# reedrosenbluth/LASS

Measured on AMD Instinct MI355X. Metric: clips/sec (10s@16kHz), higher is better.
Workload: dtype f32; 1 GPU; ResUNet30 separate() fp32, batch=16/GPU, 10s@16kHz clips, fixed precomputed condition embedding, seeded random-init weights (BASELINE configs[1]); samples_per_clip=160000, parallelism=clip-sharded x1

## Files before the change

### include/lass_hip.h

```cpp
#ifndef LASS_HIP_H
#define LASS_HIP_H

#include <stddef.h>
#include <stdint.h>

#ifdef __cplusplus
extern "C" {
#endif

typedef struct lass_ctx lass_ctx;

#define LASS_OK 0
#define LASS_ERR_ARG (-1)
#define LASS_ERR_HIP (-2)
#define LASS_ERR_STATE (-3)
#define LASS_ERR_WORKSPACE (-4)

#define LASS_F32 0
#define LASS_I64 1

#define LASS_COMPUTE_F32 0
#define LASS_COMPUTE_BF16 1
#define LASS_COMPUTE_BF16X3 2

// ... 8 lines not shown

const char* lass_last_error(const lass_ctx* ctx);

int lass_set_param(lass_ctx* ctx, const char* name, const void* data, const int64_t* shape, int ndim, int dtype);

int lass_finalize(lass_ctx* ctx, int compute_mode);

int lass_workspace_bytes(const lass_ctx* ctx, int B, int L, size_t* bytes);

int lass_separate(lass_ctx* ctx, const float* mixture, const float* condition, float* out, int B, int L,
                  void* workspace, size_t workspace_bytes, void* stream);


int lass_separate_ragged(lass_ctx* ctx, const float* mixture, const int* lengths, const float* condition, float* out,
                         int B, int L, void* workspace, size_t workspace_bytes, void* stream);
int lass_ragged_bucket(const lass_ctx* ctx, int L, int* lo, int* hi);


int lass_separate_windows(lass_ctx* ctx, const float* recording, int64_t total, const int64_t* starts, const int* keep,
                          const float* condition , float* out , int B, int W,
                          void* workspace, size_t workspace_bytes, void* stream);

int lass_separate_windows_faded(lass_ctx* ctx, const float* recording, int64_t total, const int64_t* starts, const int* keep,
                                const int* fade, const float* ramp, int F, const float* condition ,
                                float* out , int B, int W, void* workspace, size_t workspace_bytes, void* stream);

int lass_graph_stats(const lass_ctx* ctx, long* captures, long* replays);
int lass_set_graph_replay(lass_ctx* ctx, int enabled);
int lass_set_wino4_splits(lass_ctx* ctx, int splits);
int lass_set_wino4_vprep(lass_ctx* ctx, int mode);
int lass_set_head_fold(lass_ctx* ctx, int enabled);
int lass_set_head_sc_fold(lass_ctx* ctx, int enabled);
int lass_set_pw_split(lass_ctx* ctx, int enabled);
int lass_set_wino4_gemm(lass_ctx* ctx, int enabled);
int lass_set_wino4_vprep_buffer(lass_ctx* ctx, float* v, size_t floats);

int lass_separate_components(lass_ctx* ctx, const float* const* mag, const float* cos_mask, const float* sin_mask,
                             const float* condition, float* out, int B, int L, void* workspace, size_t workspace_bytes,
                             void* stream);


int lass_stft_magphase(lass_ctx* ctx, const float* wav, int B, int L, float* mag, float* cos_out, float* sin_out,
                       float* real_out, float* imag_out, void* stream);

int lass_multi_stft(lass_ctx* ctx, const float* wav, int B, int L, int hop, int n_windows, const int* win_lengths,
                    float* const* mag, float* const* cos_out, float* const* sin_out, void* stream);

int lass_stft_components(lass_ctx* ctx, const float* wav, int B, int L, int n_fft, int hop, int n_windows,
                         const int* win_lengths, float* const* mag, float* const* cos_out, float* const* sin_out,
                         void* stream);

int lass_istft(lass_ctx* ctx, const float* real, const float* imag, int B, int T, int L, float* wav,
               float* frames_ws, void* stream);
int lass_istft_nfft(lass_ctx* ctx, const float* real, const float* imag, int B, int T, int L, int n_fft, int win_length,
                    float* wav, void* stream);

int lass_film(lass_ctx* ctx, const float* condition, int B, float* shift, void* stream);
int lass_film_width(const lass_ctx* ctx);
int lass_film_offset(const lass_ctx* ctx, const char* site);
int lass_film_raw(lass_ctx* ctx, const float* condition, int B, float* film, void* stream);

int lass_convblock(lass_ctx* ctx, const char* prefix, const float* x, int B, int H, int W, const float* shift,
                   float* y, float* scratch, void* stream);

int lass_encoder_block(lass_ctx* ctx, const char* name, const float* x, int B, int H, int W, const float* shift, float* y,
                       float* pool, float* scratch, void* stream);
// ... 122 lines not shown
```

### lass_amd/_lib.py

```python
from __future__ import annotations

import ctypes
import os
from ctypes import POINTER, c_char_p, c_double, c_float, c_int, c_int64, c_long, c_size_t, c_void_p

_HERE = os.path.dirname(os.path.abspath(__file__))
LIB_PATH = os.environ.get("LASS_HIP_LIB") or os.path.join(_HERE, "csrc", "liblass_hip.so")

_lib = None

SYMBOLS = [
    ("lass_version", c_int, []),
    ("lass_create", c_int, [POINTER(c_void_p), c_int]),
    ("lass_create_stft", c_int, [POINTER(c_void_p), c_int, c_int, c_int]),
    ("lass_stft_geometry", c_int, [c_void_p, POINTER(c_int), POINTER(c_int)]),
    ("lass_create_multistft", c_int, [POINTER(c_void_p), c_int, c_int, c_int, POINTER(c_int), c_int]),
    ("lass_destroy", c_int, [c_void_p]),
    ("lass_last_error", c_char_p, [c_void_p]),
    ("lass_set_param", c_int, [c_void_p, c_char_p, c_void_p, POINTER(c_int64), c_int, c_int]),
    ("lass_finalize", c_int, [c_void_p, c_int]),
    ("lass_workspace_bytes", c_int, [c_void_p, c_int, c_int, POINTER(c_size_t)]),
    ("lass_separate", c_int, [c_void_p, c_void_p, c_void_p, c_void_p, c_int, c_int, c_void_p, c_size_t, c_void_p]),
    ("lass_separate_ragged", c_int, [c_void_p, c_void_p, c_void_p, c_void_p, c_void_p, c_int, c_int, c_void_p, c_size_t,
                                     c_void_p]),
# ... 14 lines not shown
                                         c_int, c_int, c_int, c_int, c_int, c_void_p, c_void_p]),
    ("lass_stft_magphase", c_int, [c_void_p, c_void_p, c_int, c_int, c_void_p, c_void_p, c_void_p, c_void_p,
                                   c_void_p, c_void_p]),
    ("lass_mix_at_snr", c_int, [c_void_p, c_void_p, c_void_p, c_void_p, c_void_p, c_int, c_int, c_void_p, c_void_p]),
    ("lass_decode_resample", c_int, [c_void_p, c_void_p, c_int64, c_int, c_int, c_int, c_int, c_int, c_int, c_void_p, c_int,
                                     c_void_p, c_int, c_void_p]),
    ("lass_decode_resample_planar", c_int, [c_void_p, c_void_p, c_int64, c_int, c_int, c_int, c_int, c_int, c_int, c_void_p, c_int,
                                            c_void_p, c_int, c_void_p]),
    ("lass_resample_encode", c_int, [c_void_p, c_void_p, c_int64, c_int64, c_int, c_int, c_int, c_int, c_int, c_void_p, c_int, c_int,
                                     c_void_p, c_int64, c_int, c_void_p, c_void_p]),
    ("lass_loudness", c_int, [c_void_p, c_void_p, c_int64, c_int64, c_int, c_int, c_int, c_void_p, c_int, POINTER(c_double), c_void_p,
                              c_void_p, c_void_p, c_int, c_void_p, c_size_t, c_void_p]),
    ("lass_resample_peak", c_int, [c_void_p, c_void_p, c_int64, c_int64, c_int, c_int, c_int, c_int, c_int, c_void_p, c_int, c_int,
                                   c_void_p, c_void_p]),
    ("lass_loudness_gain", c_int, [c_void_p, c_void_p, c_void_p, c_int, c_double, c_float, c_void_p, c_void_p, c_void_p]),
    ("lass_resample_encode_gain", c_int, [c_void_p, c_void_p, c_int64, c_int64, c_int, c_int, c_int, c_int, c_int, c_void_p, c_int,
                                          c_int, c_void_p, c_void_p, c_int64, c_int, c_void_p, c_void_p]),
    ("lass_resample_true_peak", c_int, [c_void_p, c_void_p, c_int64, c_int64, c_int, c_int, c_int, c_int, c_int, c_void_p, c_int, c_int,
                                        c_int, c_void_p, c_int, c_void_p, c_void_p]),
    ("lass_loudness_stats", c_int, [c_void_p, c_void_p, c_int64, c_int64, c_int, c_int, c_int, c_void_p, c_int, POINTER(c_double),
                                    c_void_p, c_void_p, c_void_p, c_int, c_void_p, c_int, c_void_p, c_size_t, c_void_p]),
    ("lass_segment_mix", c_int, [c_void_p, c_void_p, c_int, c_int, c_void_p, c_void_p, c_int, c_void_p, c_void_p, c_void_p,
                                 c_void_p, c_void_p]),
    ("lass_multi_stft", c_int, [c_void_p, c_void_p, c_int, c_int, c_int, c_int, POINTER(c_int), POINTER(c_void_p),
                                POINTER(c_void_p), POINTER(c_void_p), c_void_p]),
    ("lass_graph_stats", c_int, [c_void_p, POINTER(c_long), POINTER(c_long)]),
    ("lass_set_graph_replay", c_int, [c_void_p, c_int]),
    ("lass_set_wino4_splits", c_int, [c_void_p, c_int]),
    ("lass_set_wino4_vprep", c_int, [c_void_p, c_int]),
    ("lass_set_wino4_vprep_buffer", c_int, [c_void_p, c_void_p, c_size_t]),
    ("lass_set_head_fold", c_int, [c_void_p, c_int]),
    ("lass_set_head_sc_fold", c_int, [c_void_p, c_int]),
    ("lass_set_pw_split", c_int, [c_void_p, c_int]),
    ("lass_set_wino4_gemm", c_int, [c_void_p, c_int]),
    ("lass_separate_components", c_int, [c_void_p, POINTER(c_void_p), c_void_p, c_void_p, c_void_p, c_void_p, c_int,
                                         c_int, c_void_p, c_size_t, c_void_p]),
    ("lass_stft_components", c_int, [c_void_p, c_void_p, c_int, c_int, c_int, c_int, c_int, POINTER(c_int),
                                     POINTER(c_void_p), POINTER(c_void_p), POINTER(c_void_p), c_void_p]),
    ("lass_istft_nfft", c_int, [c_void_p, c_void_p, c_void_p, c_int, c_int, c_int, c_int, c_int, c_void_p, c_void_p]),
    ("lass_istft", c_int, [c_void_p, c_void_p, c_void_p, c_int, c_int, c_int, c_void_p, c_void_p, c_void_p]),
    ("lass_film", c_int, [c_void_p, c_void_p, c_int, c_void_p, c_void_p]),
    ("lass_film_width", c_int, [c_void_p]),
    ("lass_film_offset", c_int, [c_void_p, c_char_p]),
    ("lass_film_raw", c_int, [c_void_p, c_void_p, c_int, c_void_p, c_void_p]),
    ("lass_convblock", c_int, [c_void_p, c_char_p, c_void_p, c_int, c_int, c_int, c_void_p, c_void_p, c_void_p,
                               c_void_p]),
    ("lass_encoder_block", c_int, [c_void_p, c_char_p, c_void_p, c_int, c_int, c_int, c_void_p, c_void_p, c_void_p,
                                   c_void_p, c_void_p]),
    ("lass_front_end", c_int, [c_void_p, c_void_p, c_int, c_int, c_void_p, c_void_p, c_void_p, c_void_p, c_void_p]),
    ("lass_workspace_tensor", c_int, [c_void_p, c_int, c_int, c_char_p, POINTER(c_size_t), POINTER(c_int64),
                                      POINTER(c_int64)]),
    ("lass_upconv", c_int, [c_void_p, c_char_p, c_void_p, c_int, c_int, c_int, c_void_p, c_void_p, c_void_p]),
    ("lass_mask_apply", c_int, [c_void_p, c_void_p, c_void_p, c_void_p, c_void_p, c_int, c_int, c_int, c_void_p,
                                c_void_p, c_void_p]),
    ("lass_sdr_stats", c_int, [c_void_p, c_void_p, c_void_p, c_int, c_int, c_void_p, c_void_p]),
    ("lass_text_create", c_int, [POINTER(c_void_p), c_int]),
    ("lass_text_destroy", c_int, [c_void_p]),
    ("lass_text_last_error", c_char_p, [c_void_p]),
    ("lass_text_set_param", c_int, [c_void_p, c_char_p, c_void_p, POINTER(c_int64), c_int]),
    ("lass_text_finalize", c_int, [c_void_p]),
    ("lass_text_layers", c_int, [c_void_p]),
    ("lass_text_workspace_bytes", c_int, [c_void_p, c_int, c_int, POINTER(c_size_t)]),
    ("lass_text_encode", c_int, [c_void_p, c_void_p, c_void_p, c_int, c_int, c_void_p, c_void_p, c_void_p, c_size_t,
                                 c_void_p]),
    ("lass_audioq_create", c_int, [POINTER(c_void_p), c_int]),
    ("lass_audioq_destroy", c_int, [c_void_p]),
# ... 99 lines not shown
```

### lass_amd/csrc/api.hip

```cpp
#include <hip/hip_runtime.h>

#include <algorithm>
#include <cmath>
#include <cstdio>
#include <cstdlib>
#include <cstring>
#include <map>
#include <string>
#include <vector>

#include "../../include/lass_hip.h"
#include "ctx_parts.h"
#include "graph_cache.h"
#include "head_fold.h"
#include "kernels.h"
#include "weight_plan.h"
#include "workspace_plan.h"

namespace {

constexpr float kBnEps = 1e-5f;
constexpr int kMaxBranches = LASS_MAX_STFT_WINDOWS;

struct Site {
// ... 359 lines not shown
                            : form == BF16_DEC6U && f.up && lass_dec6u_fused_bf16_supported(p, q, uq)))
        return fail(c, LASS_ERR_STATE, rb.prefix + ": the launch arguments contradict the planned route");
    ProfScope ps(c, st, P_CONV3X3);
    HIP_TRY(c, form == BF16_ENC1 ? lass_launch_enc1_fused_bf16(p, q, st) : form == BF16_DEC6 ? lass_launch_dec6_fused_bf16(p, q, st)
                                 : lass_launch_dec6u_fused_bf16(p, q, uq, st));
    return 0;
}

int launch_routed(lass_ctx* c, const ResBlock& rb, const char* what, const ConvRoute& rt, const ConvArgs& a, const Wino4Split& sk,
                  float* vws, const Wino4Gemm& wg, hipStream_t st, const HeadScPlanes* planes = nullptr) {
    ProfScope ps(c, st, P_CONV3X3);
    bool ok = true;
    switch (rt.family) {
        case CONV_F4X4: {
            const Wino4Split s = rt.splits > 1 ? sk : Wino4Split();
            Wino4VPre vp;
            if (rt.v_from_memory) vp.v = vws;
            if (rt.head_sc_fold) {
                ok = planes && (rt.head_fold ? lass_wino4_headfold_planes_supported(a, *planes) : lass_wino4_sclogit_supported(a, *planes));
                if (ok) HIP_TRY(c, rt.head_fold ? lass_launch_wino4_headfold_planes(a, *planes, st) : lass_launch_wino4_sclogit(a, *planes, st));
                break;
            }
            if (rt.head_fold) {
                ok = lass_wino4_headfold_supported(a);
                if (ok) HIP_TRY(c, lass_launch_wino4_headfold(a, st));
                break;
            }
            if (rt.gemm) {
                ok = lass_wino4_gemm_supported(rt.kind, a, vp, wg);
                if (ok) HIP_TRY(c, lass_launch_wino4_gemm(rt.kind, a, vp, wg, st));
                break;
            }
            ok = rt.v_from_memory ? lass_wino4_vpre_supported(rt.kind, a, s) : lass_wino4_supported(rt.kind, a, s);
            if (ok) HIP_TRY(c, lass_launch_wino4(rt.kind, a, st, s, vp));
            break;
        }
        case CONV_F2X2:
            ok = lass_wino_supported(a);
            if (ok) HIP_TRY(c, lass_launch_wino(rt.kind, a, st));
            break;
        case CONV_DIRECT:
            HIP_TRY(c, lass_launch_conv(rt.kind, a, st));
            break;
        case CONV_NONE:
            ok = false;
            break;
    }
    return ok ? 0 : fail(c, LASS_ERR_STATE, rb.prefix + " " + what + ": the launch arguments contradict the planned route");
}

int run_resblock(lass_ctx* c, const ResBlock& rb, const float* x, long x_bs, int B, int H, int W, const float* shift,
                 float* a2, float* out, long out_bs, hipStream_t st, const BlockFusions& f = BlockFusions()) {
    const PreConv* pre = f.pre;
    const WeightImages& im = rb.img;
    const CatCopies *skip_out = f.skip_out, *cat_in = f.cat_in, *pool_copies = f.pool_copies;
    const float* x0 = pre ? pre->x0 : nullptr;
    const Site& s1 = c->sites[rb.s1];
    const Site& s2 = c->sites[rb.s2];
    const long HW = (long)H * W;
    ConvArgs p;
    p.in = x; p.in_bs = x_bs; p.Cin = rb.cin; p.w = im.f32(W1); p.Nw = rb.cout; p.N = rb.cout;
    p.pro_scale = c->bn_scale + s1.off; p.pro_shift = shift + s1.off; p.pro_shift_bs = c->n_shift;
    p.epi_scale = c->bn_scale + s2.off; p.epi_shift = shift + s2.off; p.epi_shift_bs = c->n_shift;
    p.out = a2; p.out_bs = rb.cout * HW; p.B = B; p.H = H; p.W = W;
    if (x0) {
        p.in = x0; p.in_bs = HW;
        p.pre_w = pre->w; p.pre_b = pre->b;
// ... 239 lines not shown

struct HeadHost {
    HeadFold hf;
    HeadScFold hsf;
    const std::vector<float>& of(WeightForm f) const {
        return f == WF_HEAD_U4 ? hf.u4 : f == WF_HEAD_WSC ? hf.wsc : f == WF_HEAD_BIAS ? hf.bias : f == WF_HEAD_SC_WT ? hsf.wt : hsf.wskip;
    }
};
int compose_head(lass_ctx* c, int Q, bool sc, HeadHost* h) {
    const ResBlock& rb = c->dec[5];
    const DecSpec& d6 = c->m.D[5];
    const int N = rb.cout, K = rb.cin;
    std::vector<float> w2, ws, bs, wa, ba, wt;
    const auto host = [&](std::vector<float>& v, const std::string& name, size_t n) -> int {
        v.resize(n);
        HIP_TRY(c, hipMemcpy(v.data(), rawp(c, name), n * sizeof(float), hipMemcpyDeviceToHost));
        return 0;
    };
    HIP_TRY(c, hipStreamSynchronize(nullptr));
    if (host(w2, rb.prefix + ".conv2.weight", (size_t)N * N * 9) || host(ws, rb.prefix + ".shortcut.weight", (size_t)N * K) ||
        host(bs, rb.prefix + ".shortcut.bias", N) || host(wa, "base.after_conv.weight", (size_t)Q * N) ||
        host(ba, "base.after_conv.bias", Q) ||
        (sc && host(wt, std::string("base.") + d6.name + ".conv1.weight", (size_t)d6.cin * d6.cout * d6.uh * d6.uw)))
        return LASS_ERR_HIP;
    if (sc) compose_head_sc_fold(ws.data(), wa.data(), wt.data(), N, d6.cout, kPreCh, Q, d6.cin, d6.uh, d6.uw, &h->hsf);
    if (!compose_head_fold(w2.data(), ws.data(), bs.data(), wa.data(), ba.data(), N, N, K, Q, &h->hf) || h->hf.u4.empty()) h->hf = HeadFold();
    return 0;
}

}

extern "C" {

int lass_version(void) { return 10900; }

const char* lass_last_error(const lass_ctx* ctx) { return ctx ? ctx->err.c_str() : g_create_err.c_str(); }

static int create_impl(lass_ctx** out, int device_id, const Geometry& geom) {
    if (!out) return LASS_ERR_ARG;
    *out = nullptr;
    if (int rc = open_device(device_id, g_create_err)) return rc;
    lass_ctx* c = new lass_ctx();
    c->device = device_id;
    c->g = geom;
    if (const char* e = getenv("LASS_FUSE_CATB")) c->cfg.fuse_catb = atoi(e) != 0;
    if (const char* e = getenv("LASS_FUSE_BLOCK")) c->cfg.fuse_block = atoi(e) != 0;
    if (const char* e = getenv("LASS_FUSE_UP")) c->cfg.fuse_up = atoi(e) != 0;
    if (const char* e = getenv("LASS_WINO4")) c->cfg.wino4_mincin = atoi(e);
    if (const char* e = getenv("LASS_WINO4_VPREP")) c->cfg.vprep_mode = std::max(0, std::min(2, atoi(e)));
    if (const char* e = getenv("LASS_HEAD_FOLD")) c->cfg.head_fold = atoi(e) != 0;
    if (const char* e = getenv("LASS_HEAD_SC_FOLD")) c->cfg.head_sc_fold = atoi(e) != 0;
    if (const char* e = getenv("LASS_PW_SPLIT")) c->cfg.pw_split = atoi(e) != 0;
    if (const char* e = getenv("LASS_WINO4_GEMM")) c->cfg.wino4_gemm = atoi(e) != 0;
    if (const char* e = getenv("LASS_SPLIT")) c->split_batch = std::max(0, std::min(2, atoi(e)));
    if (const char* e = getenv("LASS_GRAPH")) c->use_graph = atoi(e) != 0;
    c->prof.resize(P_COUNT);
    for (int i = 0; i < P_COUNT; ++i) c->prof[i].name = kProfNames[i];
    build_arch(c);
    if (hipSetDevice(device_id) != hipSuccess) {
        g_create_err = "hipSetDevice failed";
        delete c;
        return LASS_ERR_HIP;
    }
    std::vector<float2> tw2k(2048);
    for (int k = 0; k < 2048; ++k) {
        const double a = 2.0 * M_PI * k / 2048.0;
        tw2k[k] = make_float2((float)std::cos(a), (float)std::sin(a));
    }
    if (hipMalloc((void**)&c->tw2k, sizeof(float2) * 2048) != hipSuccess ||
        hipMemcpy(c->tw2k, tw2k.data(), sizeof(float2) * 2048, hipMemcpyHostToDevice) != hipSuccess) {
        g_create_err = "allocating FFT tables failed";
        delete c;
        return LASS_ERR_HIP;
    }
    *out = c;
    return 0;
}

int lass_create(lass_ctx** out, int device_id) { return create_impl(out, device_id, Geometry()); }

int lass_create_stft(lass_ctx** out, int device_id, int n_fft, int hop) {
    if (!out) return LASS_ERR_ARG;
    *out = nullptr;
    Geometry g;
    if (n_fft == 2048 && hop == 320) {
// ... 1006 lines not shown
    c->cfg.ksplit_force = splits;
    ++c->gen;
    return 0;
}

int lass_set_wino4_vprep(lass_ctx* c, int mode) {
    if (!c || mode < 0 || mode > 2) return fail(c, LASS_ERR_ARG, "lass_set_wino4_vprep: 0, 1 or 2");
    c->cfg.vprep_mode = mode;
    ++c->gen;
    return 0;
}

int lass_set_head_fold(lass_ctx* c, int enabled) {
    if (!c || (enabled != 0 && enabled != 1)) return fail(c, LASS_ERR_ARG, "lass_set_head_fold: 0 or 1");
    c->cfg.head_fold = enabled != 0;
    ++c->gen;
    return 0;
}

int lass_set_head_sc_fold(lass_ctx* c, int enabled) {
    if (!c || (enabled != 0 && enabled != 1)) return fail(c, LASS_ERR_ARG, "lass_set_head_sc_fold: 0 or 1");
    c->cfg.head_sc_fold = enabled != 0;
    ++c->gen;
    return 0;
}

int lass_set_pw_split(lass_ctx* c, int enabled) {
    if (!c || (enabled != 0 && enabled != 1)) return fail(c, LASS_ERR_ARG, "lass_set_pw_split: 0 or 1");
    c->cfg.pw_split = enabled != 0;
    ++c->gen;
    return 0;
}

int lass_set_wino4_gemm(lass_ctx* c, int enabled) {
    if (!c || (enabled != 0 && enabled != 1)) return fail(c, LASS_ERR_ARG, "lass_set_wino4_gemm: 0 or 1");
    c->cfg.wino4_gemm = enabled != 0;
    ++c->gen;
    return 0;
}

int lass_set_wino4_vprep_buffer(lass_ctx* c, float* v, size_t floats) {
    if (!c || (v && !floats)) return fail(c, LASS_ERR_ARG, "lass_set_wino4_vprep_buffer: a buffer and its size, or NULL");
    c->stage_v_user = v;
    c->stage_v_user_floats = v ? floats : 0;
    return 0;
}

int lass_graph_stats(const lass_ctx* c, long* captures, long* replays) {
    if (!c) return LASS_ERR_ARG;
    if (captures) *captures = c->g_captures;
    if (replays) *replays = c->g_replays;
    return c->use_graph ? 1 : 0;
}

int lass_separate_components(lass_ctx* c, const float* const* mag, const float* cos_mask, const float* sin_mask,
                             const float* condition, float* out, int B, int L, void* workspace, size_t workspace_bytes,
                             void* stream) {
    if (!c) return LASS_ERR_ARG;
    if (!mag || !cos_mask || !sin_mask) return fail(c, LASS_ERR_ARG, "lass_separate_components: null pointer");
    Components comp;
    for (int k = 0; k < kMaxBranches; ++k) comp.mag[k] = k < c->g.nbr ? mag[k] : nullptr;
    comp.cosv = cos_mask; comp.sinv = sin_mask;
    return separate_impl(c, nullptr, &comp, condition, out, ClipForm{B, L}, make_plan(c, B, L), workspace, workspace_bytes, stream,
                         "lass_separate_components");
}

// ... 32 lines not shown
```

### lass_amd/csrc/conv_route.h

```cpp
#pragma once
#include <stddef.h>

enum ConvKind { CONV1_ACT = 0, CONV2_IDENT = 1, CONV2_SHORTCUT = 2, TCONV_ACT = 3, CONV1_ACT_PRE = 4, CONV2_IDENT_PRE = 5 };

constexpr int kPreCh = 32;

constexpr int kWinoKC = 8;
constexpr int kWino4KC = 8;
constexpr int kWino4NXI = 36;
constexpr int kWino4VFloats = kWino4NXI * 4 * 32 * 2;
constexpr int kHeadFoldRows = 16;
constexpr int kPwGemmNB = 128;
constexpr int kPwGemmKC = 16;
constexpr int kBf16FusedTileW = 32;

inline bool lass_wino4_narrow(int H, int W) { return W % 32 == 16 && H % 32 == 0; }
inline int lass_wino4_block_tc(int H, int W) {
    if (W % 64 == 0 && H % 8 == 0) return 16;
    if (W % 32 == 0 && H % 16 == 0) return 8;
    return lass_wino4_narrow(H, W) ? 4 : 0;
}

struct ConvShape {
    int Cin = 0, N = 0, Nw = 0, H = 0, W = 0;
// ... 75 lines not shown
}
inline bool lass_dec6u_fused_bf16_shape(const ConvShape& p, const ConvShape& q, int u_cin, int u_h, int u_w) {
    return lass_dec6_fused_bf16_shape(p, q) && u_cin == 64 && u_h * 2 == p.H && u_w * 2 == p.W && p.H % 2 == 0 &&
           lass_bf16_fused_addressable(u_h, u_w);
}

constexpr int kWino4Splits = 4;

constexpr int kShortcutGemmMinCin = 256;

constexpr int kVprepMinCoutGroups = 12;

constexpr int kTconvGemmMinCin = 128;

inline bool lass_pw_split_shortcut_weights(bool f32, int cin, int cout) {
    return f32 && cin != cout && cin >= kShortcutGemmMinCin && cin % (2 * kPwGemmKC) == 0 && cout % kPwGemmNB == 0;
}
inline bool lass_pw_split_tconv_weights(bool f32, int cin, int N, int up_h) {
    return f32 && cin >= kTconvGemmMinCin && cin % (2 * kPwGemmKC) == 0 && N % kPwGemmNB == 0 && (up_h == 1 || up_h == 2) && N % (2 * up_h) == 0;
}

enum ComputeMode { MODE_F32 = 0, MODE_BF16 = 1, MODE_BF16X3 = 2 };

struct RouteCfg {
    ComputeMode mode = MODE_F32;
    bool f32() const { return mode == MODE_F32; }
    int wino4_mincin = 32;
    int ksplit_force = 0;
    int vprep_mode = 1;
    bool head_fold = true;
    bool head_sc_fold = true;
    bool wino4_gemm = true;
    bool pw_split = true;
    bool fuse_catb = true;
    bool fuse_block = true;
    bool fuse_up = true;
    bool blocked() const { return mode == MODE_BF16 && fuse_catb; }
};

struct BlockShape {
    int cin, cout;
    int width;
};

struct BlockIO {
    bool x0 = false;
    bool head = false;
    bool pool = false;
    int pool_h = 2;
    bool x_aligned = true;
    bool sc_planes = false;
    bool cat_in = false;
    bool skip_out = false;
    bool pool_copies = false;
    bool act_out = false;
    int up_cin = 0;
};

struct Wino4Images {
    bool u1f = false, u2f = false;
};
inline Wino4Images wino4_images(const RouteCfg& cfg, int cin, int cout, int width) {
    Wino4Images im;
    const int m = cfg.wino4_mincin;
    if (!cfg.f32() || m <= 0 || cin % 8 != 0 || cout % 32 != 0) return im;
    const bool level = width % 32 == 0, narrow = width % 32 == 16;
// ... 345 lines not shown
```

### lass_amd/csrc/kernels.h

```cpp
#pragma once
#include <hip/hip_runtime.h>
#include <stddef.h>
#include <stdint.h>

#include "conv_route.h"

struct ConvArgs {
    const float* in = nullptr;
    long in_bs = 0;
    int Cin = 0;
    const float* w = nullptr;
    int Nw = 0;
    const float* pro_scale = nullptr;
    const float* pro_shift = nullptr;
    int pro_shift_bs = 0;
    const float* in2 = nullptr;
    long in2_bs = 0;
    int Cin2 = 0;
    const float* w2 = nullptr;
    const float* bias = nullptr;
    const float* res = nullptr;
    long res_bs = 0;
    const float* epi_scale = nullptr;
    const float* epi_shift = nullptr;
// ... 48 lines not shown
struct Wino4Split {
    int n = 1;
    float* part = nullptr;
};

struct Wino4VPre {
    float* v = nullptr;
};

struct HeadScPlanes {
    float* skip = nullptr;
    float* up = nullptr;
    const float* w = nullptr;
};

inline ConvShape lass_conv_shape(const ConvArgs& p) {
    ConvShape s;
    s.Cin = p.Cin; s.N = p.N; s.Nw = p.Nw; s.H = p.H; s.W = p.W;
    s.Cin2 = p.Cin2; s.pool = p.pool_out != nullptr; s.pool_h = p.pool_h; s.head = p.mask_re != nullptr;
    return s;
}

hipError_t lass_launch_conv(ConvKind kind, const ConvArgs& p, hipStream_t stream);
bool lass_tconv_logits_supported(const ConvArgs& p, const HeadScPlanes& hs);
hipError_t lass_launch_tconv_logits(const ConvArgs& p, const HeadScPlanes& hs, hipStream_t stream);

bool lass_wino_supported(const ConvArgs& p);
hipError_t lass_launch_wino(ConvKind kind, const ConvArgs& p, hipStream_t stream);
hipError_t lass_launch_wino_weights(const float* w, int Cout, int Cin, float* U, hipStream_t stream);
hipError_t lass_launch_wino_shortcut_weights(const float* w, int Cout, int Cin, float* U, hipStream_t stream);

bool lass_wino4_supported(ConvKind kind, const ConvArgs& p, const Wino4Split& sk = Wino4Split());
hipError_t lass_launch_wino4(ConvKind kind, const ConvArgs& p, hipStream_t stream, const Wino4Split& sk = Wino4Split(),
                             const Wino4VPre& vp = Wino4VPre());
bool lass_wino4_vpre_supported(ConvKind kind, const ConvArgs& p, const Wino4Split& sk = Wino4Split());
hipError_t lass_launch_wino4_weights(const float* w, int Cout, int Cin, float* U, hipStream_t stream);
bool lass_wino4_headfold_supported(const ConvArgs& p);
hipError_t lass_launch_wino4_headfold(const ConvArgs& p, hipStream_t stream);
bool lass_wino4_headfold_planes_supported(const ConvArgs& p, const HeadScPlanes& hs);
hipError_t lass_launch_wino4_headfold_planes(const ConvArgs& p, const HeadScPlanes& hs, hipStream_t stream);
bool lass_wino4_sclogit_supported(const ConvArgs& p, const HeadScPlanes& hs);
hipError_t lass_launch_wino4_sclogit(const ConvArgs& p, const HeadScPlanes& hs, hipStream_t stream);

struct Wino4Gemm {
    const void* w3 = nullptr;
    float* m = nullptr;
};
bool lass_wino4_gemm_supported(ConvKind kind, const ConvArgs& p, const Wino4VPre& vp, const Wino4Gemm& g);
hipError_t lass_launch_wino4_gemm(ConvKind kind, const ConvArgs& p, const Wino4VPre& vp, const Wino4Gemm& g, hipStream_t stream);
hipError_t lass_launch_wino4_gemm_weights(const float* U, int Cout, int Cin, void* dst, hipStream_t stream);

struct PwSplitW {
    const void* w = nullptr;
};
bool lass_pw_gemm_supported(ConvKind kind, const ConvArgs& p);
hipError_t lass_launch_pw_gemm(ConvKind kind, const ConvArgs& p, hipStream_t stream, const PwSplitW& sw = PwSplitW());
hipError_t lass_launch_pw_split_weights(const float* w, int K, int Nw, void* dst, hipStream_t stream);

bool lass_bf16_supported(const ConvArgs& p);
hipError_t lass_launch_conv_bf16(ConvKind kind, const ConvArgs& p, hipStream_t stream);
hipError_t lass_launch_weights_bf16(const float* w, int Cout, int Cin, int taps, void* dst, int lo, int transposed,
                                    hipStream_t stream);

bool lass_enc1_fused_bf16_supported(const ConvArgs& p, const ConvArgs& q);
hipError_t lass_launch_enc1_fused_bf16(const ConvArgs& p, const ConvArgs& q, hipStream_t stream);
bool lass_dec6_fused_bf16_supported(const ConvArgs& p, const ConvArgs& q);
hipError_t lass_launch_dec6_fused_bf16(const ConvArgs& p, const ConvArgs& q, hipStream_t stream);
// ... 83 lines not shown
```

### lass_amd/csrc/pw_gemm_split.h

```cpp
#pragma once
#include <hip/hip_runtime.h>
#include "kernels.h"
#include "pixel_ops.h"
#include "wino_common.h"

namespace {

constexpr int NTHREADS = 256;
constexpr int NB = kPwGemmNB;
constexpr int PB = 128;
constexpr int KC = kPwGemmKC;

typedef float f32x16 __attribute__((ext_vector_type(16)));

template <bool TCONV>
__device__ __forceinline__ void acc_init(const ConvArgs& p, f32x16 (&acc)[2][2], int n0, int wn, int lane) {
#pragma unroll
    for (int i = 0; i < 2; ++i)
#pragma unroll
        for (int r = 0; r < 16; ++r) {
            const float v = TCONV ? 0.f : p.bias[n0 + wn * 64 + i * 32 + 4 * (lane >> 5) + (r & 3) + 8 * (r >> 2)];
            acc[i][0][r] = v;
            acc[i][1][r] = v;
        }
}

__device__ __forceinline__ void acc_zero(f32x16 (&acc)[2][2]) {
#pragma unroll
    for (int i = 0; i < 2; ++i)
#pragma unroll
        for (int r = 0; r < 16; ++r) acc[i][0][r] = acc[i][1][r] = 0.f;
}

template <bool TCONV>
__device__ __forceinline__ void store_tile(const ConvArgs& p, const f32x16 (&acc)[2][2], int b, int n0, unsigned p0, unsigned P, int wn,
                                           int wp, int lane) {
#pragma unroll
    for (int tp = 0; tp < 2; ++tp) {
        const unsigned pj = p0 + (unsigned)(wp * 64 + tp * 32 + (lane & 31));
        if (pj >= P) continue;
#pragma unroll
        for (int tn = 0; tn < 2; ++tn) {
            const int nb = n0 + wn * 64 + tn * 32 + 4 * (lane >> 5);
            if (!TCONV) {
                float* dst = p.out + (size_t)b * p.out_bs + pj;
#pragma unroll
                for (int r = 0; r < 16; ++r) {
                    const int n = nb + (r & 3) + 8 * (r >> 2);
                    dst[(size_t)n * P] = acc[tn][tp][r];
                }
            } else {
                const unsigned y = pj / (unsigned)p.W, x = pj - y * (unsigned)p.W;
                const int uhw = p.up_h * 2;
                const size_t oHW = (size_t)P * uhw;
                const unsigned oW = 2u * (unsigned)p.W;
                float* ob = p.out + (size_t)b * p.out_bs + (size_t)(y * p.up_h) * oW + 2u * x;
#pragma unroll
                for (int r = 0; r < 16; r += 2) {
                    const int n = nb + (r & 3) + 8 * (r >> 2);
                    const int co = n / uhw, a = (n % uhw) >> 1;
                    *reinterpret_cast<float2*>(ob + (size_t)co * oHW + (size_t)a * oW) = make_float2(acc[tn][tp][r], acc[tn][tp][r + 1]);
                }
            }
        }
    }
}

typedef __bf16 bf16x8 __attribute__((ext_vector_type(8)));
constexpr int SPLANE = (KC / 8) * NB;
static_assert(NB == PB, "both operand images have 128 columns");

typedef __bf16 bf16x2 __attribute__((ext_vector_type(2)));
typedef float f32x2 __attribute__((ext_vector_type(2)));
__device__ __forceinline__ unsigned cvt_pair(float a, float b, float& fa, float& fb) {
    const f32x2 v = {a, b};
    const unsigned u = __builtin_bit_cast(unsigned, __builtin_convertvector(v, bf16x2));
    fa = __uint_as_float(u << 16);
    fb = __uint_as_float(u & 0xffff0000u);
    return u;
}
__device__ __forceinline__ void split3(const float (&x)[8], bf16x8& h, bf16x8& m, bf16x8& l) {
    typedef unsigned u32x4 __attribute__((ext_vector_type(4)));
    u32x4 hu, mu, lu;
#pragma unroll
    for (int i = 0; i < 4; ++i) {
        float f0, f1, g0, g1;
        hu[i] = cvt_pair(x[2 * i], x[2 * i + 1], f0, f1);
        const float r0 = x[2 * i] - f0, r1 = x[2 * i + 1] - f1;
        mu[i] = cvt_pair(r0, r1, g0, g1);
        lu[i] = cvt_pair(r0 - g0, r1 - g1, f0, f1);
    }
    h = __builtin_bit_cast(bf16x8, hu);
    m = __builtin_bit_cast(bf16x8, mu);
    l = __builtin_bit_cast(bf16x8, lu);
}

}
```

### lass_amd/csrc/wino4.hip

```cpp
#include <hip/hip_runtime.h>
#include "head_fold.h"
#include "kernels.h"
#include "pixel_ops.h"
#include "wino4_transform.h"
#include "wino_common.h"

namespace {

constexpr int F_PRO = 1, F_PHASEB = 2, F_BIAS = 4, F_RES = 8, F_EPIACT = 16, F_PRECONV = 64, F_RESPRE = 128, F_MASK = 1024;
constexpr int F_SPLITK = 2048;
constexpr int F_SCLOGIT = 8192;
constexpr int F_VPRE = 4096;
constexpr int NTHREADS = 256;
constexpr int KC = kWino4KC;
constexpr int NXI = kWino4NXI;
constexpr int U_F = NXI * 256;
constexpr int V_F = kWino4VFloats;

typedef float f32x2v __attribute__((ext_vector_type(2)));


template <int TC, int FLAGS>
__global__ __launch_bounds__(NTHREADS, 2) void wino4_kernel(ConvArgs p) {
    const Wino4Split sk;
    const Wino4VPre vp;
    const HeadScPlanes hs;
#include "wino4_body.h"
}
template <int TC, int FLAGS0>
__global__ __launch_bounds__(NTHREADS, 2) void wino4_splitk_kernel(ConvArgs p, Wino4Split sk) {
    constexpr int FLAGS = FLAGS0 | F_SPLITK;
    const Wino4VPre vp;
    const HeadScPlanes hs;
#include "wino4_body.h"
}
template <int TC, int FLAGS0>
__global__ __launch_bounds__(NTHREADS, 2) void wino4_vpre_kernel(ConvArgs p, Wino4Split sk, Wino4VPre vp) {
    constexpr int FLAGS = FLAGS0 | F_VPRE;
    const HeadScPlanes hs;
#include "wino4_body.h"
}
template <int TC, int FLAGS0>
__global__ __launch_bounds__(NTHREADS, 2) void wino4_sclogit_kernel(ConvArgs p, HeadScPlanes hs) {
    constexpr int FLAGS = FLAGS0 | F_SCLOGIT;
    const Wino4Split sk;
// ... 216 lines not shown
    hipLaunchKernelGGL((wino4_splitk_kernel<4, MAIN>), dim3((unsigned)((long)p.gx * p.gy * p.B * sk.n)), dim3(NTHREADS), 0, stream, p, sk);
    if (hipError_t e = hipGetLastError()) return e;
    const long items = (long)p.B * p.N * (p.H / 2) * (p.W / 4);
    hipLaunchKernelGGL((wino4_combine_kernel<COMB>), dim3((unsigned)((items + 255) / 256)), dim3(256), 0, stream, p, sk);
    return hipGetLastError();
}

}

bool lass_wino4_supported(ConvKind kind, const ConvArgs& p, const Wino4Split& sk) {
    if (!lass_wino4_shape(kind, lass_conv_shape(p), sk.n) || !p.w_wino4 || (sk.n != 1 && !sk.part)) return false;
    switch (kind) {
        case CONV1_ACT:
            return true;
        case CONV1_ACT_PRE:
            return p.pre_w && p.pre_b;
        case CONV2_IDENT_PRE:
            return p.res && p.pre_w && p.pre_b;
        case CONV2_IDENT:
            return p.res != nullptr;
        case CONV2_SHORTCUT:
            if (!(p.in2 && p.w2 && p.bias)) return false;
            return !p.mask_re || (p.W + 1 == p.mask_nbins && p.mask_w && p.mask_b && p.mask_mag && p.mask_cos && p.mask_sin && p.mask_im &&
                                  p.mask_T > 0 && p.mask_T <= p.H);
        default:
            return false;
    }
}

bool lass_wino4_vpre_supported(ConvKind kind, const ConvArgs& p, const Wino4Split& sk) {
    return lass_wino4_vpre_shape(kind, lass_conv_shape(p), sk.n) && lass_wino4_supported(kind, p, sk);
}

hipError_t lass_launch_wino4(ConvKind kind, const ConvArgs& p, hipStream_t stream, const Wino4Split& sk, const Wino4VPre& vp) {
    if (!lass_wino4_supported(kind, p, sk) || !p.in || (!p.out && !p.mask_re)) return hipErrorInvalidValue;
    if (vp.v) {
        if (!lass_wino4_vpre_supported(kind, p, sk)) return hipErrorInvalidValue;
        if (kind == CONV1_ACT) {
            if (!p.pro_scale || !p.pro_shift || !p.epi_scale || !p.epi_shift) return hipErrorInvalidValue;
            return launch_wino4_vpre<F_EPIACT>(p, sk, vp, stream);
        }
        return launch_wino4_vpre<F_RES>(p, sk, vp, stream);
    }
    switch (kind) {
        case CONV1_ACT:
        case CONV1_ACT_PRE:
            if (!p.pro_scale || !p.pro_shift || !p.epi_scale || !p.epi_shift) return hipErrorInvalidValue;
            if (sk.n > 1) return launch_wino4_split<F_PRO, F_EPIACT>(p, sk, stream);
            return kind == CONV1_ACT ? launch_wino4<F_PRO | F_EPIACT>(p, stream) : launch_wino4<F_PRO | F_EPIACT | F_PRECONV>(p, stream);
        case CONV2_IDENT:
            if (sk.n > 1) return launch_wino4_split<0, F_RES>(p, sk, stream);
            return launch_wino4<F_RES>(p, stream);
        case CONV2_IDENT_PRE:
            return launch_wino4<F_RES | F_RESPRE>(p, stream);
        case CONV2_SHORTCUT:
            return p.mask_re ? launch_wino4<F_PHASEB | F_BIAS | F_MASK>(p, stream) : launch_wino4<F_PHASEB | F_BIAS>(p, stream);
        default:
            return hipErrorInvalidValue;
    }
}

bool lass_wino4_headfold_supported(const ConvArgs& p) {
    return lass_wino4_headfold_shape(lass_conv_shape(p)) && p.in && p.w_wino4 && p.in2 && p.w2 && p.bias && p.W + 1 == p.mask_nbins &&
           p.mask_mag && p.mask_cos && p.mask_sin && p.mask_re && p.mask_im && p.mask_T > 0 && p.mask_T <= p.H;
}

hipError_t lass_launch_wino4_headfold(const ConvArgs& p, hipStream_t stream) {
    if (!lass_wino4_headfold_supported(p)) return hipErrorInvalidValue;
    return launch_wino4_headfold_tc<16>(p, stream);
}

bool lass_wino4_headfold_planes_supported(const ConvArgs& p, const HeadScPlanes& hs) {
    return lass_wino4_headfold_supported(p) && hs.skip && hs.up;
}

hipError_t lass_launch_wino4_headfold_planes(const ConvArgs& p, const HeadScPlanes& hs, hipStream_t stream) {
    if (!lass_wino4_headfold_planes_supported(p, hs)) return hipErrorInvalidValue;
    return launch_wino4_headfold_planes_tc<16>(p, hs, stream);
}

bool lass_wino4_sclogit_supported(const ConvArgs& p, const HeadScPlanes& hs) {
    return lass_wino4_supported(CONV2_IDENT_PRE, p) && lass_wino4_block_tc(p.H, p.W) == 16 && p.in && p.out && hs.skip && hs.w;
}

hipError_t lass_launch_wino4_sclogit(const ConvArgs& p, const HeadScPlanes& hs, hipStream_t stream) {
    if (!lass_wino4_sclogit_supported(p, hs)) return hipErrorInvalidValue;
    return launch_wino4_sclogit_tc<16>(p, hs, stream);
}
// ... 7 lines not shown
```

### lass_amd/csrc/wino4_body.h

```cpp
    constexpr bool PRO = (FLAGS & F_PRO) != 0, EPI = (FLAGS & F_EPIACT) != 0, SC = (FLAGS & F_PHASEB) != 0;
    constexpr bool PRE = (FLAGS & F_PRECONV) != 0;
    constexpr bool RESPRE = (FLAGS & F_RESPRE) != 0;
    constexpr bool MASK = (FLAGS & F_MASK) != 0;
    constexpr bool RES = (FLAGS & F_RES) != 0;
    static_assert(!SC || (FLAGS & F_BIAS) != 0, "the shortcut conv has a bias");
    static_assert(!PRE || PRO, "pre_conv is folded into the prologue's affine");
    static_assert(!RESPRE || ((FLAGS & F_RES) != 0 && !SC && !EPI), "conv2 with the identity residual");
    static_assert(!MASK || SC, "the output head sits behind decoder_block6's conv2 + shortcut");
    static_assert(!RES || (!SC && !EPI), "conv2 with a residual in place of the fused shortcut");
    constexpr bool SPLIT = (FLAGS & F_SPLITK) != 0;
    static_assert(!SPLIT || (FLAGS & ~(F_SPLITK | F_PRO | F_VPRE)) == 0, "a split launch has a prologue at most");
    constexpr bool VPRE = (FLAGS & F_VPRE) != 0;
    static_assert(!VPRE || (FLAGS & ~(F_VPRE | F_SPLITK | F_EPIACT | F_RES)) == 0, "conv1 / identity conv2 / split share: the prologue ran in the prep launch");
    constexpr bool SCL = (FLAGS & F_SCLOGIT) != 0;
    static_assert(!SCL || (FLAGS == (F_RES | F_RESPRE | F_SCLOGIT) && TC == 16), "the skip's logits: encoder_block1.conv2 on the 8 x 64 blocks");
    constexpr int TR = 32 / TC;
    constexpr int OR_ = 4 * TR, OC = 4 * TC;
    constexpr int NCO = 32;
    __shared__ __attribute__((aligned(16))) float lds[U_F + V_F + 2 * NCO + (MASK ? 100 : 0) + (SCL ? 96 : 0)];
    float* lu = lds;
    float* lv = lds + U_F;
    float* lds_es = lv + V_F;
    float* lds_eh = lds_es + NCO;
    float* lds_mw = lds_eh + NCO;

    const int tid = threadIdx.x;
    const int lane = tid & 63, wave = __builtin_amdgcn_readfirstlane(tid >> 6);
    const int wco = wave >> 1, wwt = wave & 1;
    int bx_, by_, b, ks = 0;
    if constexpr (SPLIT) {
        const unsigned lin = blockIdx.x, ngrp = (unsigned)(p.gx * p.B * sk.n);
        unsigned grp;
        if (p.xcd_map) {
            const unsigned j = lin >> 3;
            grp = (lin & 7u) * (ngrp >> 3) + j / (unsigned)p.gy;
            by_ = (int)(j % (unsigned)p.gy);
        } else {
            grp = lin / (unsigned)p.gy;
            by_ = (int)(lin % (unsigned)p.gy);
        }
        ks = (int)(grp % (unsigned)sk.n);
        const unsigned xz = grp / (unsigned)sk.n;
// ... 177 lines not shown
#pragma unroll
            for (int r = 0; r < 4; ++r) w4[r] = lds_mw[q * 32 + wco * 16 + kq * 4 + r];
#pragma unroll
            for (int a = 0; a < 4; ++a) {
                float4 o;
                float* op = &o.x;
#pragma unroll
                for (int c = 0; c < 4; ++c) {
                    const f32x4 v = ysp[a * 4 + c];
                    op[c] = fmaf(v[3], w4[3], fmaf(v[2], w4[2], fmaf(v[1], w4[1], v[0] * w4[0])));
                }
                *reinterpret_cast<float4*>(part + ((wco * 4 + kq) * 3 + q) * 512 + ot * 16 + a * 4) = o;
            }
        }
    }
    if constexpr (RES && !RESPRE) {
        float4 rv[4][4];
#pragma unroll
        for (int r = 0; r < 4; ++r) {
            const float* rr = p.res + (size_t)b * p.res_bs + (size_t)(n0 + wco * 16 + kq * 4 + r) * HW + (size_t)min(oy, p.H - 4) * p.W + ox;
#pragma unroll
            for (int a = 0; a < 4; ++a) rv[r][a] = *reinterpret_cast<const float4*>(rr + (size_t)a * p.W);
        }
#pragma unroll
        for (int r = 0; r < 4; ++r)
#pragma unroll
            for (int a = 0; a < 4; ++a) {
                ysp[a * 4 + 0][r] += rv[r][a].x;
                ysp[a * 4 + 1][r] += rv[r][a].y;
                ysp[a * 4 + 2][r] += rv[r][a].z;
                ysp[a * 4 + 3][r] += rv[r][a].w;
            }
    }
    if constexpr (SC) {
        const float* x2 = p.in2 + (size_t)b * p.in2_bs + (size_t)min(oy, p.H - 4) * p.W + ox;
        const float* wsc = p.w2 + n0 + wco * 16 + l15;
        const int nks = p.Cin2 / 4;
        constexpr int NSB = 4;
        float4 xb[NSB][4];
        float wa[NSB];
        auto ldk = [&](int ks, int buf) {
            const float* xp = x2 + (size_t)(4 * ks + kq) * HW;
#pragma unroll
            for (int a = 0; a < 4; ++a) xb[buf][a] = *reinterpret_cast<const float4*>(xp + (size_t)a * p.W);
            wa[buf] = wsc[(size_t)(4 * ks + kq) * p.Nw];
        };
        auto mmk = [&](int buf) {
#pragma unroll
            for (int a = 0; a < 4; ++a) {
                ysp[a * 4 + 0] = __builtin_amdgcn_mfma_f32_16x16x4f32(wa[buf], xb[buf][a].x, ysp[a * 4 + 0], 0, 0, 0);
                ysp[a * 4 + 1] = __builtin_amdgcn_mfma_f32_16x16x4f32(wa[buf], xb[buf][a].y, ysp[a * 4 + 1], 0, 0, 0);
                ysp[a * 4 + 2] = __builtin_amdgcn_mfma_f32_16x16x4f32(wa[buf], xb[buf][a].z, ysp[a * 4 + 2], 0, 0, 0);
                ysp[a * 4 + 3] = __builtin_amdgcn_mfma_f32_16x16x4f32(wa[buf], xb[buf][a].w, ysp[a * 4 + 3], 0, 0, 0);
            }
        };
        ldk(0, 0);
        ldk(1, 1);
        ldk(2, 2);
        for (int ks = 0; ks < nks; ks += NSB) {
#pragma unroll
            for (int u = 0; u < NSB; ++u) {
                ldk(min(ks + u + 3, nks - 1), (u + 3) % NSB);
                __builtin_amdgcn_sched_barrier(0);
                mmk(u);
                __builtin_amdgcn_sched_barrier(0);
            }
        }
// ... 106 lines not shown
```

### lass_amd/engine.py

```python
from __future__ import annotations

from ctypes import byref, c_char_p, c_double, c_int, c_int64, c_size_t, c_void_p
from typing import Dict, Optional

import numpy as np
import torch

from . import _alloc, _lib, arch, longform


def _ptr(t: Optional[torch.Tensor]):
    return c_void_p(t.data_ptr()) if t is not None else c_void_p(0)


def _stream(device) -> c_void_p:
    return c_void_p(torch.cuda.current_stream(device).cuda_stream)


class Engine:

    def __init__(self, device="cuda:0", multistft=None, stft=None):
        if stft is not None:
            if multistft is not None:
                raise ValueError("stft=(n_fft, hop) is ResUNet30's geometry: the multi-STFT model has its own (n_fft, hop 160)")
# ... 725 lines not shown
            if tuple(peak.shape) != (B,):
                raise _lib.LassError(f"peak must have shape ({B},)")
        gain = _alloc.empty(B, dtype=torch.float32, device=self.device)
        limited = _alloc.empty(B, dtype=torch.int32, device=self.device)
        rc = self.lib.lass_loudness_gain(self.ctx, _ptr(loudness), _ptr(peak), B, float("nan") if target is None else float(target),
                                         0.0 if ceiling is None else float(ceiling), _ptr(gain), _ptr(limited), _stream(self.device))
        _lib.check(self.ctx, rc, "lass_loudness_gain")
        return gain, limited

    def segment_mix(self, waveforms: torch.Tensor, mix_num: torch.Tensor, comp_db: torch.Tensor, noise_db: torch.Tensor):
        waveforms = self._dev(waveforms)
        B, L = waveforms.shape
        mix_num = mix_num.to(device=self.device, dtype=torch.int32).contiguous()
        comp_db = comp_db.to(device=self.device, dtype=torch.float32).contiguous()
        noise_db = noise_db.to(device=self.device, dtype=torch.float32).contiguous()
        if mix_num.shape != (B,) or noise_db.shape != (B,) or comp_db.dim() != 2 or comp_db.shape[0] != B:
            raise ValueError("segment_mix: mix_num (B), comp_db (B, max_mix_num - 1), noise_db (B) expected")
        mixture, segment = _alloc.empty_like(waveforms), _alloc.empty_like(waveforms)
        scratch = _alloc.empty(B, 4, dtype=torch.float64, device=self.device)
        rc = self.lib.lass_segment_mix(self.ctx, _ptr(waveforms), B, L, _ptr(mix_num), _ptr(comp_db), int(comp_db.shape[1]),
                                       _ptr(noise_db), _ptr(mixture), _ptr(segment), _ptr(scratch), _stream(self.device))
        _lib.check(self.ctx, rc, "lass_segment_mix")
        return mixture, segment

    def graph_stats(self):
        from ctypes import c_long
        cap, rep = c_long(), c_long()
        on = self.lib.lass_graph_stats(self.ctx, byref(cap), byref(rep))
        return bool(on), cap.value, rep.value

    def set_graph_replay(self, on: bool):
        _lib.check(self.ctx, self.lib.lass_set_graph_replay(self.ctx, 1 if on else 0), "lass_set_graph_replay")

    def set_profiling(self, on: bool):
        self.lib.lass_set_profiling(self.ctx, 1 if on else 0)

    def profile(self, reset: bool = True) -> Dict[str, tuple]:
        out = {}
        for i in range(self.lib.lass_profile_count(self.ctx)):
            name, ms, n = c_char_p(), c_double(), c_int()
            self.lib.lass_profile_get(self.ctx, i, byref(name), byref(ms), byref(n))
            out[name.value.decode()] = (ms.value, n.value)
        if reset:
            self.lib.lass_profile_reset(self.ctx)
        return out


def arch_cond() -> int:
    return 512


_ENGINES: Dict[int, Engine] = {}


def get_engine(device) -> Engine:
    device = torch.device(device)
    idx = device.index if device.index is not None else torch.cuda.current_device()
    if idx not in _ENGINES:
        _ENGINES[idx] = Engine(torch.device("cuda", idx))
    return _ENGINES[idx]
```

Before: 1184 clips/s.

## Run wino4 fused shortcut phase on bf16x3 split MFMA with LDS exchange

Adds an F_SCSPLIT variant of the fused 1x1 shortcut inside the wino4 conv2+shortcut kernel. Instead of fp32 16x16x4 MFMAs, it splits weights and inputs into three bf16 parts and issues six 16x16x32 bf16 MFMAs per product, keeping near-fp32 accuracy with higher matrix throughput. Paired waves exchange their split operands through LDS with barriers, so loads are shared across the two output-channel halves. The shared split3 helper moves into a common header, and the path is on by default (sc_split=true) when Cin2 is a multiple of 32. In exchange it adds conversion arithmetic, LDS traffic and synchronisation.

Result: no change. 1187 clips/s, median of 6 (+0.3%).

```diff
diff --git a/include/lass_hip.h b/include/lass_hip.h
--- a/include/lass_hip.h
+++ b/include/lass_hip.h
@@ -64,6 +64,7 @@
 int lass_set_head_fold(lass_ctx* ctx, int enabled);
 int lass_set_head_sc_fold(lass_ctx* ctx, int enabled);
 int lass_set_pw_split(lass_ctx* ctx, int enabled);
+int lass_set_sc_split(lass_ctx* ctx, int enabled);
 int lass_set_wino4_gemm(lass_ctx* ctx, int enabled);
 int lass_set_wino4_vprep_buffer(lass_ctx* ctx, float* v, size_t floats);
 
diff --git a/lass_amd/_lib.py b/lass_amd/_lib.py
--- a/lass_amd/_lib.py
+++ b/lass_amd/_lib.py
@@ -70,6 +70,7 @@
     ("lass_set_head_fold", c_int, [c_void_p, c_int]),
     ("lass_set_head_sc_fold", c_int, [c_void_p, c_int]),
     ("lass_set_pw_split", c_int, [c_void_p, c_int]),
+    ("lass_set_sc_split", c_int, [c_void_p, c_int]),
     ("lass_set_wino4_gemm", c_int, [c_void_p, c_int]),
     ("lass_separate_components", c_int, [c_void_p, POINTER(c_void_p), c_void_p, c_void_p, c_void_p, c_void_p, c_int,
                                          c_int, c_void_p, c_size_t, c_void_p]),
diff --git a/lass_amd/csrc/api.hip b/lass_amd/csrc/api.hip
--- a/lass_amd/csrc/api.hip
+++ b/lass_amd/csrc/api.hip
@@ -415,7 +415,7 @@
                 break;
             }
             ok = rt.v_from_memory ? lass_wino4_vpre_supported(rt.kind, a, s) : lass_wino4_supported(rt.kind, a, s);
-            if (ok) HIP_TRY(c, lass_launch_wino4(rt.kind, a, st, s, vp));
+            if (ok) HIP_TRY(c, lass_launch_wino4(rt.kind, a, st, s, vp, c->cfg.sc_split));
             break;
         }
         case CONV_F2X2:
@@ -721,7 +721,7 @@
 
 extern "C" {
 
-int lass_version(void) { return 10900; }
+int lass_version(void) { return 11000; }
 
 const char* lass_last_error(const lass_ctx* ctx) { return ctx ? ctx->err.c_str() : g_create_err.c_str(); }
 
@@ -740,6 +740,7 @@
     if (const char* e = getenv("LASS_HEAD_FOLD")) c->cfg.head_fold = atoi(e) != 0;
     if (const char* e = getenv("LASS_HEAD_SC_FOLD")) c->cfg.head_sc_fold = atoi(e) != 0;
     if (const char* e = getenv("LASS_PW_SPLIT")) c->cfg.pw_split = atoi(e) != 0;
+    if (const char* e = getenv("LASS_SC_SPLIT")) c->cfg.sc_split = atoi(e) != 0;
     if (const char* e = getenv("LASS_WINO4_GEMM")) c->cfg.wino4_gemm = atoi(e) != 0;
     if (const char* e = getenv("LASS_SPLIT")) c->split_batch = std::max(0, std::min(2, atoi(e)));
     if (const char* e = getenv("LASS_GRAPH")) c->use_graph = atoi(e) != 0;
@@ -1812,6 +1813,13 @@
     return 0;
 }
 
+int lass_set_sc_split(lass_ctx* c, int enabled) {
+    if (!c || (enabled != 0 && enabled != 1)) return fail(c, LASS_ERR_ARG, "lass_set_sc_split: 0 or 1");
+    c->cfg.sc_split = enabled != 0;
+    ++c->gen;
+    return 0;
+}
+
 int lass_set_wino4_gemm(lass_ctx* c, int enabled) {
     if (!c || (enabled != 0 && enabled != 1)) return fail(c, LASS_ERR_ARG, "lass_set_wino4_gemm: 0 or 1");
     c->cfg.wino4_gemm = enabled != 0;
diff --git a/lass_amd/csrc/bf16_split.h b/lass_amd/csrc/bf16_split.h
--- /dev/null
+++ b/lass_amd/csrc/bf16_split.h
@@ -0,0 +1,33 @@
+#pragma once
+#include <hip/hip_runtime.h>
+
+namespace {
+
+typedef __bf16 bf16x8 __attribute__((ext_vector_type(8)));
+
+typedef __bf16 bf16x2 __attribute__((ext_vector_type(2)));
+typedef float f32x2 __attribute__((ext_vector_type(2)));
+__device__ __forceinline__ unsigned cvt_pair(float a, float b, float& fa, float& fb) {
+    const f32x2 v = {a, b};
+    const unsigned u = __builtin_bit_cast(unsigned, __builtin_convertvector(v, bf16x2));
+    fa = __uint_as_float(u << 16);
+    fb = __uint_as_float(u & 0xffff0000u);
+    return u;
+}
+__device__ __forceinline__ void split3(const float (&x)[8], bf16x8& h, bf16x8& m, bf16x8& l) {
+    typedef unsigned u32x4 __attribute__((ext_vector_type(4)));
+    u32x4 hu, mu, lu;
+#pragma unroll
+    for (int i = 0; i < 4; ++i) {
+        float f0, f1, g0, g1;
+        hu[i] = cvt_pair(x[2 * i], x[2 * i + 1], f0, f1);
+        const float r0 = x[2 * i] - f0, r1 = x[2 * i + 1] - f1;
+        mu[i] = cvt_pair(r0, r1, g0, g1);
+        lu[i] = cvt_pair(r0 - g0, r1 - g1, f0, f1);
+    }
+    h = __builtin_bit_cast(bf16x8, hu);
+    m = __builtin_bit_cast(bf16x8, mu);
+    l = __builtin_bit_cast(bf16x8, lu);
+}
+
+}
diff --git a/lass_amd/csrc/conv_route.h b/lass_amd/csrc/conv_route.h
--- a/lass_amd/csrc/conv_route.h
+++ b/lass_amd/csrc/conv_route.h
@@ -131,6 +131,7 @@
     bool head_sc_fold = true;
     bool wino4_gemm = true;
     bool pw_split = true;
+    bool sc_split = true;
     bool fuse_catb = true;
     bool fuse_block = true;
     bool fuse_up = true;
diff --git a/lass_amd/csrc/kernels.h b/lass_amd/csrc/kernels.h
--- a/lass_amd/csrc/kernels.h
+++ b/lass_amd/csrc/kernels.h
@@ -104,7 +104,7 @@
 
 bool lass_wino4_supported(ConvKind kind, const ConvArgs& p, const Wino4Split& sk = Wino4Split());
 hipError_t lass_launch_wino4(ConvKind kind, const ConvArgs& p, hipStream_t stream, const Wino4Split& sk = Wino4Split(),
-                             const Wino4VPre& vp = Wino4VPre());
+                             const Wino4VPre& vp = Wino4VPre(), bool sc_split = false);
 bool lass_wino4_vpre_supported(ConvKind kind, const ConvArgs& p, const Wino4Split& sk = Wino4Split());
 hipError_t lass_launch_wino4_weights(const float* w, int Cout, int Cin, float* U, hipStream_t stream);
 bool lass_wino4_headfold_supported(const ConvArgs& p);
diff --git a/lass_amd/csrc/pw_gemm_split.h b/lass_amd/csrc/pw_gemm_split.h
--- a/lass_amd/csrc/pw_gemm_split.h
+++ b/lass_amd/csrc/pw_gemm_split.h
@@ -1,5 +1,6 @@
 #pragma once
 #include <hip/hip_runtime.h>
+#include "bf16_split.h"
 #include "kernels.h"
 #include "pixel_ops.h"
 #include "wino_common.h"
@@ -66,33 +67,7 @@
     }
 }
 
-typedef __bf16 bf16x8 __attribute__((ext_vector_type(8)));
 constexpr int SPLANE = (KC / 8) * NB;
 static_assert(NB == PB, "both operand images have 128 columns");
 
-typedef __bf16 bf16x2 __attribute__((ext_vector_type(2)));
-typedef float f32x2 __attribute__((ext_vector_type(2)));
-__device__ __forceinline__ unsigned cvt_pair(float a, float b, float& fa, float& fb) {
-    const f32x2 v = {a, b};
-    const unsigned u = __builtin_bit_cast(unsigned, __builtin_convertvector(v, bf16x2));
-    fa = __uint_as_float(u << 16);
-    fb = __uint_as_float(u & 0xffff0000u);
-    return u;
 }
-__device__ __forceinline__ void split3(const float (&x)[8], bf16x8& h, bf16x8& m, bf16x8& l) {
-    typedef unsigned u32x4 __attribute__((ext_vector_type(4)));
-    u32x4 hu, mu, lu;
-#pragma unroll
-    for (int i = 0; i < 4; ++i) {
-        float f0, f1, g0, g1;
-        hu[i] = cvt_pair(x[2 * i], x[2 * i + 1], f0, f1);
-        const float r0 = x[2 * i] - f0, r1 = x[2 * i + 1] - f1;
-        mu[i] = cvt_pair(r0, r1, g0, g1);
-        lu[i] = cvt_pair(r0 - g0, r1 - g1, f0, f1);
-    }
-    h = __builtin_bit_cast(bf16x8, hu);
-    m = __builtin_bit_cast(bf16x8, mu);
-    l = __builtin_bit_cast(bf16x8, lu);
-}
-
-}
diff --git a/lass_amd/csrc/wino4.hip b/lass_amd/csrc/wino4.hip
--- a/lass_amd/csrc/wino4.hip
+++ b/lass_amd/csrc/wino4.hip
@@ -1,4 +1,5 @@
 #include <hip/hip_runtime.h>
+#include "bf16_split.h"
 #include "head_fold.h"
 #include "kernels.h"
 #include "pixel_ops.h"
@@ -11,6 +12,7 @@
 constexpr int F_SPLITK = 2048;
 constexpr int F_SCLOGIT = 8192;
 constexpr int F_VPRE = 4096;
+constexpr int F_SCSPLIT = 16384;
 constexpr int NTHREADS = 256;
 constexpr int KC = kWino4KC;
 constexpr int NXI = kWino4NXI;
@@ -293,7 +295,7 @@
     return lass_wino4_vpre_shape(kind, lass_conv_shape(p), sk.n) && lass_wino4_supported(kind, p, sk);
 }
 
-hipError_t lass_launch_wino4(ConvKind kind, const ConvArgs& p, hipStream_t stream, const Wino4Split& sk, const Wino4VPre& vp) {
+hipError_t lass_launch_wino4(ConvKind kind, const ConvArgs& p, hipStream_t stream, const Wino4Split& sk, const Wino4VPre& vp, bool sc_split) {
     if (!lass_wino4_supported(kind, p, sk) || !p.in || (!p.out && !p.mask_re)) return hipErrorInvalidValue;
     if (vp.v) {
         if (!lass_wino4_vpre_supported(kind, p, sk)) return hipErrorInvalidValue;
@@ -315,6 +317,8 @@
         case CONV2_IDENT_PRE:
             return launch_wino4<F_RES | F_RESPRE>(p, stream);
         case CONV2_SHORTCUT:
+            if (sc_split && p.Cin2 % 32 == 0)
+                return p.mask_re ? launch_wino4<F_PHASEB | F_BIAS | F_MASK | F_SCSPLIT>(p, stream) : launch_wino4<F_PHASEB | F_BIAS | F_SCSPLIT>(p, stream);
             return p.mask_re ? launch_wino4<F_PHASEB | F_BIAS | F_MASK>(p, stream) : launch_wino4<F_PHASEB | F_BIAS>(p, stream);
         default:
             return hipErrorInvalidValue;
diff --git a/lass_amd/csrc/wino4_body.h b/lass_amd/csrc/wino4_body.h
--- a/lass_amd/csrc/wino4_body.h
+++ b/lass_amd/csrc/wino4_body.h
@@ -8,6 +8,8 @@
     static_assert(!RESPRE || ((FLAGS & F_RES) != 0 && !SC && !EPI), "conv2 with the identity residual");
     static_assert(!MASK || SC, "the output head sits behind decoder_block6's conv2 + shortcut");
     static_assert(!RES || (!SC && !EPI), "conv2 with a residual in place of the fused shortcut");
+    constexpr bool SCSPLIT = (FLAGS & F_SCSPLIT) != 0;
+    static_assert(!SCSPLIT || SC, "the split form of the shortcut phase");
     constexpr bool SPLIT = (FLAGS & F_SPLITK) != 0;
     static_assert(!SPLIT || (FLAGS & ~(F_SPLITK | F_PRO | F_VPRE)) == 0, "a split launch has a prologue at most");
     constexpr bool VPRE = (FLAGS & F_VPRE) != 0;
@@ -251,7 +253,81 @@
                 ysp[a * 4 + 3][r] += rv[r][a].w;
             }
     }
-    if constexpr (SC) {
+    if constexpr (SC && SCSPLIT) {
+        bf16x8* sx = reinterpret_cast<bf16x8*>(lds);
+        lds_barrier();
+        const float* x2 = p.in2 + (size_t)b * p.in2_bs + (size_t)(8 * kq) * HW + (size_t)(min(oy, p.H - 4) + wco) * p.W + ox;
+        const float* wsc = p.w2 + (size_t)(8 * kq) * p.Nw + n0 + wco * 16 + l15;
+        const int nst = p.Cin2 / 32;
+        float4 xr[2][8];
+        float wr[8];
+        auto ldrow = [&](int st, int h) {
+            const float* xp = x2 + (size_t)(32 * st) * HW + (size_t)(2 * h) * p.W;
+#pragma unroll
+            for (int j = 0; j < 8; ++j) xr[h][j] = *reinterpret_cast<const float4*>(xp + (size_t)j * HW);
+        };
+        auto ldw = [&](int st) {
+#pragma unroll
+            for (int j = 0; j < 8; ++j) wr[j] = wsc[(size_t)(32 * st + j) * p.Nw];
+        };
+        auto scphase = [&](auto wc) {
+            constexpr int WCO = decltype(wc)::value;
+            ldw(0);
+            ldrow(0, 0);
+            for (int st = 0; st < nst; ++st) {
+                bf16x8 wp[3];
+                split3(wr, wp[0], wp[1], wp[2]);
+                const int stn = min(st + 1, nst - 1);
+                ldw(stn);
+                constexpr int WP[6] = {2, 0, 1, 1, 0, 0}, XP[6] = {0, 2, 1, 0, 1, 0};
+#pragma unroll
+                for (int h = 0; h < 2; ++h) {
+                    if (h == 0)
+                        ldrow(st, 1);
+                    else
+                        ldrow(stn, 0);
+                    __builtin_amdgcn_sched_barrier(0);
+#pragma unroll
+                    for (int g = 0; g < 2; ++g) {
+                        bf16x8 xp[2][3];
+#pragma unroll
+                        for (int cc = 0; cc < 2; ++cc) {
+                            float x[8];
+#pragma unroll
+                            for (int j = 0; j < 8; ++j) {
+                                const float4 v = xr[h][j];
+                                x[j] = g == 0 ? (cc == 0 ? v.x : v.y) : (cc == 0 ? v.z : v.w);
+                            }
+                            split3(x, xp[cc][0], xp[cc][1], xp[cc][2]);
+#pragma unroll
+                            for (int pc = 0; pc < 3; ++pc) sx[((((g * 2 + wwt) * 2 + WCO) * 2 + cc) * 3 + pc) * 64 + lane] = xp[cc][pc];
+                            f32x4 d = ysp[(2 * h + WCO) * 4 + 2 * g + cc];
+#pragma unroll
+                            for (int t = 0; t < 6; ++t) d = __builtin_amdgcn_mfma_f32_16x16x32_bf16(wp[WP[t]], xp[cc][XP[t]], d, 0, 0, 0);
+                            ysp[(2 * h + WCO) * 4 + 2 * g + cc] = d;
+                        }
+                        lds_barrier();
+#pragma unroll
+                        for (int cc = 0; cc < 2; ++cc)
+#pragma unroll
+                            for (int pc = 0; pc < 3; ++pc) xp[cc][pc] = sx[((((g * 2 + wwt) * 2 + (WCO ^ 1)) * 2 + cc) * 3 + pc) * 64 + lane];
+#pragma unroll
+                        for (int t = 0; t < 6; ++t)
+#pragma unroll
+                            for (int cc = 0; cc < 2; ++cc) {
+                                f32x4& d = ysp[(2 * h + (WCO ^ 1)) * 4 + 2 * g + cc];
+                                d = __builtin_amdgcn_mfma_f32_16x16x32_bf16(wp[WP[t]], xp[cc][XP[t]], d, 0, 0, 0);
+                            }
+                    }
+                }
+            }
+        };
+        if (wco == 0)
+            scphase(std::integral_constant<int, 0>());
+        else
+            scphase(std::integral_constant<int, 1>());
+    }
+    if constexpr (SC && !SCSPLIT) {
         const float* x2 = p.in2 + (size_t)b * p.in2_bs + (size_t)min(oy, p.H - 4) * p.W + ox;
         const float* wsc = p.w2 + n0 + wco * 16 + l15;
         const int nks = p.Cin2 / 4;
diff --git a/lass_amd/engine.py b/lass_amd/engine.py
--- a/lass_amd/engine.py
+++ b/lass_amd/engine.py
@@ -781,6 +781,9 @@
     def set_graph_replay(self, on: bool):
         _lib.check(self.ctx, self.lib.lass_set_graph_replay(self.ctx, 1 if on else 0), "lass_set_graph_replay")
 
+    def set_sc_split(self, on: bool):
+        _lib.check(self.ctx, self.lib.lass_set_sc_split(self.ctx, 1 if on else 0), "lass_set_sc_split")
+
     def set_profiling(self, on: bool):
         self.lib.lass_set_profiling(self.ctx, 1 if on else 0)
 
```
